# 0kam/alproj

Hardware: AMD Instinct MI355X
Metric: Gpoints/s projected (pinhole + Brown-Conrady, single pose) over the 100M-vertex DSM; CMA-ES iterations/s in `cma` (higher is better)
Workload: dtype f32

## Files before the change

### alproj_amd/csrc/alp_cma.hip

```cpp
#include "alp_points_internal.h"
#include "alp_sampler.h"

#include <cmath>

namespace {

using namespace alp;

constexpr int CMA_MAX_D = SAMPLER_MAX_D;
constexpr int CMA_MAX_P = 4096;
constexpr int CMA_MAX_STARTS = 1024;
constexpr int64_t CMA_MAX_TOTAL = 65536;
constexpr int TELL_THREADS = 256;
constexpr int JACOBI_MAX_SWEEPS = 40;
constexpr double CMA_EPS = 1e-8;
constexpr double CMA_SIGMA_MAX = 1e32;

struct CmaState {
    double mean[CMA_MAX_D], ps[CMA_MAX_D], pc[CMA_MAX_D], d[CMA_MAX_D];
    double C[CMA_MAX_D * CMA_MAX_D], B[CMA_MAX_D * CMA_MAX_D];
    double BD[CMA_MAX_D * CMA_MAX_D];
    double sigma;
    long long g;
    unsigned k0, k1;
};

struct CmaHyper {
    int D, P, mu, dmax, K;
    double mu_eff, c1, cmu, cc, c_sigma, d_sigma, chi_n, cm, sum_w;
};

struct ExpandArgs {
    double tmpl[ALP_NPARAM];
    double lo[CMA_MAX_D], hi[CMA_MAX_D];
    int idx[CMA_MAX_D];
    double origin[3];
};

template <typename T, int DMAX, bool LF>
__global__ __launch_bounds__(256) void cma_generation_kernel(SamplerArgs a0, ExpandArgs e, const CmaState *__restrict__ states, long long P,
                                                             long long total, double *__restrict__ x_out, double *__restrict__ cand_out,
                                                             PoseRec<T> *__restrict__ recs, long long lf_off) {
    const long long cand = ((long long)blockIdx.x * blockDim.x + threadIdx.x) >> 6;
    if (cand >= total) return;
    const long long start = cand / P, draw = cand - start * P;
    const CmaState *st = states + start;
    const int lane = (int)(threadIdx.x & 63);
    SamplerArgs a = a0;
#pragma unroll
    for (int i = 0; i < DMAX; ++i)
        if (i < a.D) a.mean[i] = st->mean[i];
    a.sigma = st->sigma;
    a.gen = (unsigned)st->g;
    a.k0 = st->k0;
    a.k1 = st->k1;
    const double *BD = st->BD;
    double z[DMAX], x[DMAX];
#pragma unroll
    for (int j = 0; j < DMAX; ++j) z[j] = 0.0;
    int accepted = -1;
    for (int base = 0; base < a.n_max && accepted < 0; base += 64) {
        const int t = base + lane;
        bool ok = false;
        if (t < a.n_max) {
            draw_normals<DMAX>(z, a.D, (unsigned)t, (unsigned)draw, a.gen, a.k0, a.k1);
            ok = make_x<DMAX, false>(a, BD, z, x);
        }
        const unsigned long long m = __ballot(ok);
        if (m) accepted = base + __ffsll((long long)m) - 1;
    }
    const int t_final = accepted >= 0 ? accepted : a.n_max;
    if (lane != (t_final & 63)) return;
    draw_normals<DMAX>(z, a.D, (unsigned)t_final, (unsigned)draw, a.gen, a.k0, a.k1);
    make_x<DMAX, true>(a, BD, z, x);
    double prm[ALP_NPARAM];
    for (int k = 0; k < ALP_NPARAM; ++k) prm[k] = e.tmpl[k];
#pragma unroll
    for (int i = 0; i < DMAX; ++i)
        if (i < a.D) {
            double xi = x[i];
            if (accepted < 0 && a.bounded) xi = fmin(fmax(xi, a.lower[i]), a.upper[i]);
            x_out[cand * a.D + i] = xi;
            prm[e.idx[i]] = xi * (e.hi[i] - e.lo[i]) + e.lo[i];
        }
    for (int k = 0; k < ALP_NPARAM; ++k) cand_out[cand * ALP_NPARAM + k] = prm[k];
    double g[POSE_WORDS];
    fold_pose_hd(prm, e.origin, g);
    for (int k = 0; k < POSE_WORDS; ++k) recs[cand].v[k] = (T)g[k];
    if (LF) {
        double lf[POSE_WORDS];
        lens_free_from_general_hd(g, lf);
        for (int k = 0; k < POSE_WORDS; ++k) recs[lf_off + cand].v[k] = (T)lf[k];
    }
}

__device__ __forceinline__ void circle_pair(int m, int r, int k, int *p, int *q) {
    const int a = k == 0 ? m - 1 : (r + k) % (m - 1);
    const int b = (r - k + (m - 1)) % (m - 1);
    *p = a < b ? a : b;
    *q = a < b ? b : a;
}

__device__ void jacobi_eigen(int D, double *C, double *B, double *d2, double *A, double *A2, double *V, double *V2, double *self_,
                             double *oth, double *dlt, int *partner, int *rotated, int *nrot) {
    const int tid = threadIdx.x;
    const int DD = D * D;
    for (int e = tid; e < DD; e += blockDim.x) {
        const int i = e / D, j = e % D;
        double s = 0;
        for (int k = 0; k < D; ++k) s += B[k * D + i] * B[k * D + j];
        A2[e] = s;
    }
    __syncthreads();
    for (int e = tid; e < DD; e += blockDim.x) {
        const int i = e / D, j = e % D;
        double s = 0;
        for (int k = 0; k < D; ++k) s += B[i * D + k] * ((k == j ? 1.5 : 0.0) - 0.5 * A2[k * D + j]);
        V2[e] = s;
    }
    __syncthreads();
    for (int e = tid; e < DD; e += blockDim.x) B[e] = V2[e];
    __syncthreads();
    for (int e = tid; e < DD; e += blockDim.x) {
        const int i = e / D, j = e % D;
        double s = 0;
        for (int k = 0; k < D; ++k) s += C[i * D + k] * B[k * D + j];
        A2[e] = s;
    }
    __syncthreads();
    for (int e = tid; e < DD; e += blockDim.x) {
        const int i = e / D, j = e % D;
        if (i <= j) {
            double s = 0;
            for (int k = 0; k < D; ++k) s += B[k * D + i] * A2[k * D + j];
            A[i * D + j] = s;
            A[j * D + i] = s;
        }
        V[e] = i == j ? 1.0 : 0.0;
    }
    __syncthreads();
    const int m = (D + 1) & ~1;
    for (int sweep = 0; sweep < JACOBI_MAX_SWEEPS && m >= 2; ++sweep) {
        if (tid == 0) *nrot = 0;
        __syncthreads();
        for (int r = 0; r < m - 1; ++r) {
            if (tid < m / 2) {
                int p, q;
                circle_pair(m, r, tid, &p, &q);
                if (q < D) {
                    const double app = A[p * D + p], aqq = A[q * D + q], apq = A[p * D + q];
                    const double g = 100.0 * fabs(apq);
                    double c = 1.0, s = 0.0, t = 0.0;
                    const bool rot = apq != 0.0 && !(fabs(app) + g == fabs(app) && fabs(aqq) + g == fabs(aqq));
                    if (rot) {
                        const double theta = (aqq - app) / (2.0 * apq);
                        if (fabs(theta) > 1e150) t = 0.5 / theta;
                        else {
                            t = 1.0 / (fabs(theta) + sqrt(theta * theta + 1.0));
                            if (theta < 0) t = -t;
                        }
                        c = 1.0 / sqrt(t * t + 1.0);
                        s = t * c;
                        *nrot = 1;
                    }
                    partner[p] = q; partner[q] = p;
                    self_[p] = c; self_[q] = c;
                    oth[p] = -s; oth[q] = s;
                    dlt[p] = -t * apq; dlt[q] = t * apq;
                    rotated[p] = rotated[q] = rot;
                } else if (p < D) {
                    partner[p] = p; self_[p] = 1.0; oth[p] = 0.0; dlt[p] = 0.0; rotated[p] = 0;
                }
            }
            __syncthreads();
            for (int e = tid; e < DD; e += blockDim.x) {
                const int i = e / D, j = e % D;
                double v;
                if (i == j) v = A[e] + dlt[i];
                else if (partner[i] == j && rotated[i]) v = 0.0;
                else {
                    const int lo = i < j ? i : j, hi = i < j ? j : i;
                    const int plo = partner[lo], phi = partner[hi];
                    v = self_[hi] * A[lo * D + hi];
                    if (oth[hi] != 0.0) v += oth[hi] * A[lo * D + phi];
                    v *= self_[lo];
                    if (oth[lo] != 0.0) {
                        double w = self_[hi] * A[plo * D + hi];
                        if (oth[hi] != 0.0) w += oth[hi] * A[plo * D + phi];
                        v += oth[lo] * w;
                    }
                }
                A2[e] = v;
                double u = V[i * D + j] * self_[j];
                if (oth[j] != 0.0) u += V[i * D + partner[j]] * oth[j];
                V2[e] = u;
            }
            __syncthreads();
            for (int e = tid; e < DD; e += blockDim.x) {
                A[e] = A2[e];
                V[e] = V2[e];
            }
            __syncthreads();
        }
        if (*nrot == 0) break;
        __syncthreads();
    }
    for (int e = tid; e < DD; e += blockDim.x) {
        const int i = e / D, j = e % D;
        double s = 0;
        for (int k = 0; k < D; ++k) s += B[i * D + k] * V[k * D + j];
        V2[e] = s;
    }
    for (int i = tid; i < D; i += blockDim.x) d2[i] = A[i * D + i];
    __syncthreads();
    for (int e = tid; e < DD; e += blockDim.x) B[e] = V2[e];
    __syncthreads();
}

template <bool TELL>
__global__ __launch_bounds__(TELL_THREADS) void cma_tell_kernel(CmaHyper h, CmaState *__restrict__ states, const double *__restrict__ weights,
                                                                const double *__restrict__ X_all, const double *__restrict__ sums_all,
                                                                const double *__restrict__ vals_all, double *__restrict__ loss_all,
                                                                int *__restrict__ order_all, double *__restrict__ ys_all,
                                                                double *__restrict__ wio_all) {
    const long long k = blockIdx.x, kP = k * h.P, kPD = kP * h.D;
    CmaState *__restrict__ st = states + k;
    const double *__restrict__ X = X_all + kPD;
    const double *__restrict__ sums = sums_all ? sums_all + kP : nullptr;
    const double n_total = sums_all ? sums_all[(long long)h.K * h.P] : 0.0;
    const double *__restrict__ vals = vals_all ? vals_all + kP : nullptr;
    double *__restrict__ loss_out = loss_all + kP;
    int *__restrict__ order_out = order_all + kP;
    double *__restrict__ ys = ys_all + kPD;
    double *__restrict__ wio = wio_all + kP;
    constexpr int M = CMA_MAX_D * CMA_MAX_D;
    __shared__ double C[M], B[M], A[M], A2[M], V[M], V2[M];
    __shared__ double mean[CMA_MAX_D], d[CMA_MAX_D], yw[CMA_MAX_D], ps[CMA_MAX_D], pc[CMA_MAX_D], d2[CMA_MAX_D];
    __shared__ double self_[CMA_MAX_D], oth[CMA_MAX_D], dlt[CMA_MAX_D];
    __shared__ int partner[CMA_MAX_D], rotated[CMA_MAX_D];
    __shared__ int nrot;
    __shared__ double sig, hsig;
    const int tid = threadIdx.x, D = h.D, P = h.P, DD = D * D;
    for (int e = tid; e < DD; e += blockDim.x) {
        C[e] = st->C[e];
        B[e] = st->B[e];
    }
    for (int i = tid; i < D; i += blockDim.x) {
        mean[i] = st->mean[i];
        d[i] = st->d[i];
        ps[i] = st->ps[i];
        pc[i] = st->pc[i];
    }
    if (tid == 0) sig = st->sigma;
    __syncthreads();
    if (TELL) {
        const long long g = st->g + 1;
        for (int i = tid; i < P; i += blockDim.x) loss_out[i] = vals ? vals[i] : sums[i] / n_total;
        __syncthreads();
        for (int i = tid; i < P; i += blockDim.x) {
            double ki = loss_out[i];
            if (ki != ki) ki = INFINITY;
            int r = 0;
            for (int j = 0; j < P; ++j) {
                double kj = loss_out[j];
                if (kj != kj) kj = INFINITY;
                r += (kj < ki) || (kj == ki && j < i);
            }
            order_out[r] = i;
        }
        __syncthreads();
        const double sigma = sig;
        for (int e = tid; e < P * D; e += blockDim.x) {
            const int r = e / D, j = e % D;
            ys[e] = (X[(long long)order_out[r] * D + j] - mean[j]) / sigma;
        }
        __syncthreads();
        for (int j = tid; j < D; j += blockDim.x) {
            double s = 0.0;
            for (int r = 0; r < h.mu; ++r) s = s + ys[(long long)r * D + j] * weights[r];
            yw[j] = s;
        }
        __syncthreads();
        const double cs = h.c_sigma, cmsig = h.cm * sigma;
        for (int e = tid; e < DD; e += blockDim.x) {
            const int i = e / D, j = e % D;
            double s = 0.0;
            for (int k = 0; k < D; ++k) s += (B[i * D + k] / d[k]) * B[j * D + k];
            A[e] = s;
        }
        for (int j = tid; j < D; j += blockDim.x) mean[j] = mean[j] + cmsig * yw[j];
        __syncthreads();
        const double sq_ps = sqrt(cs * (2.0 - cs) * h.mu_eff);
        for (int i = tid; i < D; i += blockDim.x) {
            double s = 0.0;
            for (int k = 0; k < D; ++k) s += A[i * D + k] * yw[k];
            ps[i] = (1.0 - cs) * ps[i] + sq_ps * s;
        }
        __syncthreads();
        if (tid == 0) {
            double nn = 0.0;
            for (int k = 0; k < D; ++k) nn += ps[k] * ps[k];
            const double norm_ps = sqrt(nn);
            double s2 = sig * exp((cs / h.d_sigma) * (norm_ps / h.chi_n - 1.0));
            sig = s2 < CMA_SIGMA_MAX ? s2 : CMA_SIGMA_MAX;
            const double h_left = norm_ps / sqrt(1.0 - pow(1.0 - cs, (double)(2 * (g + 1))));
            const double h_right = (1.4 + 2.0 / (double)(D + 1)) * h.chi_n;
            hsig = h_left < h_right ? 1.0 : 0.0;
        }
        __syncthreads();
        const double h_sigma = hsig, cc = h.cc;
        const double sq_pc = h_sigma * sqrt(cc * (2.0 - cc) * h.mu_eff);
        for (int i = tid; i < D; i += blockDim.x) pc[i] = (1.0 - cc) * pc[i] + sq_pc * yw[i];
        for (int r = tid; r < P; r += blockDim.x) {
            const double wr = weights[r];
            if (wr >= 0) {
                wio[r] = wr * 1.0;
            } else {
                double nn = 0.0;
                for (int i = 0; i < D; ++i) {
                    double s = 0.0;
                    for (int k = 0; k < D; ++k) s += ys[(long long)r * D + k] * A[i * D + k];
                    nn += s * s;
                }
                const double nrm = sqrt(nn);
                wio[r] = wr * ((double)D / (nrm * nrm + CMA_EPS));
            }
        }
        __syncthreads();
        const double delta_h = (1.0 - h_sigma) * cc * (2.0 - cc);
        const double c1 = h.c1, cmu = h.cmu;
        const double coef = 1.0 + c1 * delta_h - c1 - cmu * h.sum_w;
        for (int e = tid; e < DD; e += blockDim.x) {
            const int i = e / D, j = e % D;
            double rmu = 0.0;
            for (int r = 0; r < P; ++r) rmu += (ys[(long long)r * D + i] * wio[r]) * ys[(long long)r * D + j];
            A2[e] = coef * C[e] + c1 * (pc[i] * pc[j]) + cmu * rmu;
        }
        __syncthreads();
        for (int e = tid; e < DD; e += blockDim.x) C[e] = A2[e];
        if (tid == 0) st->g = g;
        __syncthreads();
    }
    for (int e = tid; e < DD; e += blockDim.x) {
        const int i = e / D, j = e % D;
        A2[e] = (C[i * D + j] + C[j * D + i]) / 2.0;
    }
    __syncthreads();
    for (int e = tid; e < DD; e += blockDim.x) C[e] = A2[e];
    __syncthreads();
    jacobi_eigen(D, C, B, d2, A, A2, V, V2, self_, oth, dlt, partner, rotated, &nrot);
    for (int i = tid; i < D; i += blockDim.x) d[i] = sqrt(d2[i] < 0 ? CMA_EPS : d2[i]);
    __syncthreads();
    for (int e = tid; e < DD; e += blockDim.x) {
        const int i = e / D, j = e % D;
        double s = 0.0;
        for (int k = 0; k < D; ++k) s += (B[i * D + k] * (d[k] * d[k])) * B[j * D + k];
        st->C[e] = s;
        st->B[e] = B[e];
    }
    for (int e = tid; e < h.dmax * h.dmax; e += blockDim.x) {
        const int i = e / h.dmax, j = e % h.dmax;
        st->BD[e] = (i < D && j < D) ? B[i * D + j] * d[j] : 0.0;
    }
    for (int i = tid; i < D; i += blockDim.x) {
        st->d[i] = d[i];
        if (TELL) {
            st->mean[i] = mean[i];
            st->ps[i] = ps[i];
            st->pc[i] = pc[i];
        }
    }
    if (TELL && tid == 0) st->sigma = sig;
}

}

struct alp_cma {
    alp_points *pts = nullptr;
    CmaHyper hy{};
    SamplerArgs sa{};
    ExpandArgs ex{};
    std::vector<uint64_t> seeds;
    bool lens_free = false, shared_pose = false;
    void *dev = nullptr;
    CmaState *st = nullptr;
    double *w = nullptr, *X = nullptr, *cand = nullptr, *loss = nullptr, *ys = nullptr, *wio = nullptr, *vals = nullptr;
    int *order = nullptr;
    bool pending = false;
    bool have_last = false;
    int64_t rows() const { return (int64_t)hy.K * hy.P; }
};

namespace alp {
void cma_points_gone(alp_cma_t *h) { h->pts = nullptr; }
}

namespace {

void fill_state(const alp_cma *h, int k, CmaState *s, const double *mean, double sigma, const double *C, const double *ps, const double *pc,
                int64_t g) {
    const int D = h->hy.D;
    memset(s, 0, sizeof(*s));
    for (int i = 0; i < D; ++i) {
        s->mean[i] = mean[i];
        s->ps[i] = ps[i];
        s->pc[i] = pc[i];
        s->d[i] = 1.0;
        s->B[i * D + i] = 1.0;
    }
    for (int e = 0; e < D * D; ++e) s->C[e] = C[e];
    s->sigma = sigma;
    s->g = g;
    s->k0 = (unsigned)h->seeds[(size_t)k];
    s->k1 = (unsigned)(h->seeds[(size_t)k] >> 32);
}

int upload_states(alp_cma *h, int k0, int n, const CmaState *s) {
    hipStream_t st = ctx().stream;
    ALP_HIP(hipMemcpyAsync(h->st + k0, s, (size_t)n * sizeof(CmaState), hipMemcpyHostToDevice, st));
    hipLaunchKernelGGL(cma_tell_kernel<false>, dim3(n), dim3(TELL_THREADS), 0, st, h->hy, h->st + k0, (const double *)h->w,
                       (const double *)h->X, (const double *)nullptr, (const double *)nullptr, h->loss, h->order, h->ys, h->wio);
    ALP_HIP(hipGetLastError());
    ALP_HIP(hipStreamSynchronize(st));
    return ALP_OK;
}

int usable(alp_cma *h, const char *what) {
    if (int rc = require_init()) return rc;
    if (!h) return fail(ALP_EINVAL, "%s: handle is NULL", what);
    if (h->pending) return fail(ALP_ESTATE, "%s: generations are enqueued; call alp_cma_wait first", what);
    return ALP_OK;
}

template <typename T, int DMAX>
void launch_generation(alp_cma *h, unsigned grid, hipStream_t st) {
    alp_points *p = h->pts;
    PoseRec<T> *recs = (PoseRec<T> *)p->cand_dev;
    if (h->lens_free)
        hipLaunchKernelGGL((cma_generation_kernel<T, DMAX, true>), dim3(grid), dim3(256), 0, st, h->sa, h->ex, (const CmaState *)h->st,
                           (long long)h->hy.P, (long long)h->rows(), h->X, h->cand, recs, (long long)p->cand_cap);
    else
        hipLaunchKernelGGL((cma_generation_kernel<T, DMAX, false>), dim3(grid), dim3(256), 0, st, h->sa, h->ex, (const CmaState *)h->st,
                           (long long)h->hy.P, (long long)h->rows(), h->X, h->cand, recs, (long long)p->cand_cap);
}

template <typename T>
void launch_generation_t(alp_cma *h, unsigned grid, hipStream_t st) {
    if (h->hy.dmax == 12) launch_generation<T, 12>(h, grid, st);
    else if (h->hy.dmax == 24) launch_generation<T, 24>(h, grid, st);
    else launch_generation<T, 32>(h, grid, st);
}

}

extern "C" {

int alp_cma_create_starts(alp_points_t *pts, const double tmpl[ALP_NPARAM], const int32_t *target_idx, int D, const double *lower,
                          const double *upper, int64_t P, int K, const double *weights, const double hyper[ALP_CMA_NHYPER],
                          int n_max_resampling, const uint64_t *seeds, alp_cma_t **out) {
    if (int rc = require_init()) return rc;
    ALP_REQUIRE(out, "out is NULL");
    *out = nullptr;
    ALP_REQUIRE(pts && tmpl && target_idx && lower && upper && weights && hyper && seeds, "NULL argument");
    ALP_REQUIRE(D >= 1 && D <= CMA_MAX_D, "D must be in [1, 32]");
    ALP_REQUIRE(P >= 1 && P <= CMA_MAX_P, "P must be in [1, 4096]");
    ALP_REQUIRE(K >= 1 && K <= CMA_MAX_STARTS, "K must be in [1, 1024]");
    ALP_REQUIRE((int64_t)K * P <= CMA_MAX_TOTAL, "K * P must be at most 65536");
    ALP_REQUIRE(n_max_resampling >= 0 && n_max_resampling <= (1 << 20), "n_max_resampling out of range");
    if (!pts->uo) return fail(ALP_ESTATE, "alp_cma_create: observed uv not set");
    for (int i = 0; i < D; ++i) {
        ALP_REQUIRE(target_idx[i] >= 0 && target_idx[i] < ALP_NPARAM, "target index out of range");
        ALP_REQUIRE(target_idx[i] != 21 && target_idx[i] != 22, "w and h cannot be targets (every candidate must share the image size)");
    }
    const int mu = (int)hyper[0];
    ALP_REQUIRE(mu >= 0 && mu <= P, "mu out of range");
    alp_cma *h = new alp_cma();
    h->pts = pts;
    const int dmax = D <= 12 ? 12 : (D <= 24 ? 24 : 32);
    h->hy = CmaHyper{D, (int)P, mu, dmax, K, hyper[1], hyper[2], hyper[3], hyper[4], hyper[5], hyper[6], hyper[7], hyper[8], hyper[9]};
    h->seeds.assign(seeds, seeds + K);
    memset(&h->sa, 0, sizeof(h->sa));
    for (int i = 0; i < D; ++i) {
        h->sa.lower[i] = 0.0;
        h->sa.upper[i] = 1.0;
    }
    h->sa.D = D;
    h->sa.n_max = n_max_resampling;
    h->sa.bounded = 1;
    memset(&h->ex, 0, sizeof(h->ex));
    for (int k = 0; k < ALP_NPARAM; ++k) h->ex.tmpl[k] = tmpl[k];
    for (int i = 0; i < D; ++i) {
        h->ex.idx[i] = target_idx[i];
        h->ex.lo[i] = lower[i];
        h->ex.hi[i] = upper[i];
    }
    memcpy(h->ex.origin, pts->origin, sizeof(h->ex.origin));
    bool lf = !getenv("ALP_POP_NO_LENS_FREE");
    for (int k = 9; k <= 20 && lf; ++k) lf = tmpl[k] == 0.0;
    for (int i = 0; i < D && lf; ++i) lf = !(target_idx[i] >= 9 && target_idx[i] <= 20);
    bool shared = P > 1 && !lf;
    for (int i = 0; i < D && shared; ++i) shared = target_idx[i] >= 7 && target_idx[i] <= 20;
    h->lens_free = lf;
    h->shared_pose = shared;
    const int64_t R = (int64_t)K * P;
    const size_t sz_state = round_up((int64_t)K * sizeof(CmaState), 256), sz_w = round_up(P * 8, 256), sz_p = round_up(R * 8, 256),
                 sz_pd = round_up(R * D * 8, 256), sz_cand = round_up(R * ALP_NPARAM * 8, 256), sz_ord = round_up(R * 4, 256);
    int rc = ALP_OK;
    if (hipMalloc(&h->dev, sz_state + sz_w + 3 * sz_p + 2 * sz_pd + sz_cand + sz_ord) != hipSuccess) rc = fail(ALP_EHIP, "alp_cma_create: hipMalloc failed");
    if (!rc) {
        char *q = (char *)h->dev;
        h->st = (CmaState *)q; q += sz_state;
        h->w = (double *)q; q += sz_w;
        h->loss = (double *)q; q += sz_p;
        h->wio = (double *)q; q += sz_p;
        h->vals = (double *)q; q += sz_p;
        h->X = (double *)q; q += sz_pd;
        h->ys = (double *)q; q += sz_pd;
        h->cand = (double *)q; q += sz_cand;
        h->order = (int *)q;
        if (hipMemcpy(h->w, weights, (size_t)P * 8, hipMemcpyHostToDevice) != hipSuccess) rc = fail(ALP_EHIP, "alp_cma_create: weights upload failed");
    }
    if (!rc) rc = points_pop_reserve(pts, R);
    if (!rc) {
        std::vector<double> mean(D, 0.5), C((size_t)D * D, 0.0), zero(D, 0.0);
        for (int i = 0; i < D; ++i) C[(size_t)i * D + i] = 1.0;
        std::vector<CmaState> s((size_t)K);
        for (int k = 0; k < K; ++k) fill_state(h, k, &s[(size_t)k], mean.data(), 1.0, C.data(), zero.data(), zero.data(), 0);
        rc = upload_states(h, 0, K, s.data());
    }
    if (rc) {
        if (h->dev) hipFree(h->dev);
        delete h;
        return rc;
    }
    pts->loops.push_back(h);
    *out = h;
    return ALP_OK;
}

int alp_cma_create(alp_points_t *pts, const double tmpl[ALP_NPARAM], const int32_t *target_idx, int D, const double *lower,
                   const double *upper, int64_t P, const double *weights, const double hyper[ALP_CMA_NHYPER], int n_max_resampling,
                   uint64_t seed, alp_cma_t **out) {
    return alp_cma_create_starts(pts, tmpl, target_idx, D, lower, upper, P, 1, weights, hyper, n_max_resampling, &seed, out);
}

int alp_cma_destroy(alp_cma_t *h) {
    if (!h) return ALP_OK;
    if (ctx().ready) hipStreamSynchronize(ctx().stream);
    if (h->pts) {
        h->pts->loop_pending = false;
        auto &v = h->pts->loops;
        for (size_t i = 0; i < v.size(); ++i)
            if (v[i] == h) {
                v.erase(v.begin() + (long)i);
                break;
            }
    }
    if (h->dev) hipFree(h->dev);
    delete h;
    return ALP_OK;
}

int alp_cma_set_state_at(alp_cma_t *h, int k, const double *mean, double sigma, const double *C, const double *p_sigma, const double *pc,
                         int64_t generation) {
    if (int rc = usable(h, "alp_cma_set_state")) return rc;
    ALP_REQUIRE(k >= 0 && k < h->hy.K, "start index out of range");
    ALP_REQUIRE(mean && C && p_sigma && pc, "NULL argument");
    ALP_REQUIRE(sigma > 0, "sigma must be positive");
    ALP_REQUIRE(generation >= 0, "generation is negative");
    CmaState s;
    fill_state(h, k, &s, mean, sigma, C, p_sigma, pc, generation);
    return upload_states(h, k, 1, &s);
}

int alp_cma_set_state(alp_cma_t *h, const double *mean, double sigma, const double *C, const double *p_sigma, const double *pc,
                      int64_t generation) {
    return alp_cma_set_state_at(h, 0, mean, sigma, C, p_sigma, pc, generation);
}

int alp_cma_get_state_at(alp_cma_t *h, int k, double *mean, double *sigma, double *C, double *p_sigma, double *pc, int64_t *generation,
                         double *B, double *Dvec) {
    if (int rc = usable(h, "alp_cma_get_state")) return rc;
    ALP_REQUIRE(k >= 0 && k < h->hy.K, "start index out of range");
    CmaState s;
    ALP_HIP(hipMemcpyAsync(&s, h->st + k, sizeof(s), hipMemcpyDeviceToHost, ctx().stream));
    ALP_HIP(hipStreamSynchronize(ctx().stream));
    const int D = h->hy.D;
    for (int i = 0; i < D; ++i) {
        if (mean) mean[i] = s.mean[i];
        if (p_sigma) p_sigma[i] = s.ps[i];
        if (pc) pc[i] = s.pc[i];
        if (Dvec) Dvec[i] = s.d[i];
    }
    for (int e = 0; e < D * D; ++e) {
        if (C) C[e] = s.C[e];
        if (B) B[e] = s.B[e];
    }
    if (sigma) *sigma = s.sigma;
    if (generation) *generation = s.g;
    return ALP_OK;
}

int alp_cma_get_state(alp_cma_t *h, double *mean, double *sigma, double *C, double *p_sigma, double *pc, int64_t *generation, double *B,
                      double *Dvec) {
    return alp_cma_get_state_at(h, 0, mean, sigma, C, p_sigma, pc, generation, B, Dvec);
}

int alp_cma_run(alp_cma_t *h, int64_t generations, int loss_kind, double f_scale) {
    if (int rc = usable(h, "alp_cma_run")) return rc;
    ALP_REQUIRE(generations >= 0, "generations is negative");
    ALP_REQUIRE(loss_kind == ALP_LOSS_MEAN_DIST || loss_kind == ALP_LOSS_HUBER, "unknown loss_kind");
    alp_points *p = h->pts;
    if (!p) return fail(ALP_ESTATE, "alp_cma_run: the point set of this device loop has been destroyed");
    if (p->pending_P > 0 || p->loop_pending)
        return fail(ALP_ESTATE, "alp_cma_run: the point set has an evaluation enqueued that has not been waited for");
    if (generations == 0) return ALP_OK;
    const int64_t R = h->rows();
    if (int rc = points_pop_reserve(p, R)) return rc;
    const unsigned grid = (unsigned)((R * 64 + 255) / 256);
    const bool batched = h->hy.K > 1;
    hipStream_t st = ctx().stream;
    h->pending = true;
    p->loop_pending = true;
    for (int64_t g = 0; g < generations; ++g) {
        if (p->precision == ALP_F64) launch_generation_t<double>(h, grid, st);
        else launch_generation_t<float>(h, grid, st);
        ALP_HIP(hipGetLastError());
        if (int rc = popeval_launch(p, R, loss_kind, f_scale, h->lens_free, h->shared_pose, batched, h->cand)) return rc;
        hipLaunchKernelGGL(cma_tell_kernel<true>, dim3(h->hy.K), dim3(TELL_THREADS), 0, st, h->hy, h->st, (const double *)h->w,
                           (const double *)h->X, (const double *)p->sums_dev, (const double *)nullptr, h->loss, h->order, h->ys, h->wio);
        ALP_HIP(hipGetLastError());
    }
    h->have_last = true;
    return ALP_OK;
}

int alp_cma_wait(alp_cma_t *h) {
    if (int rc = require_init()) return rc;
    ALP_REQUIRE(h, "handle is NULL");
    if (!h->pending) return fail(ALP_ESTATE, "alp_cma_wait: nothing enqueued");
    h->pending = false;
    if (h->pts) h->pts->loop_pending = false;
    ALP_HIP(hipStreamSynchronize(ctx().stream));
    return ALP_OK;
}

int alp_cma_tell_host(alp_cma_t *h, const double *X, const double *losses, int32_t *order_out) {
    if (int rc = usable(h, "alp_cma_tell_host")) return rc;
    ALP_REQUIRE(X && losses, "NULL argument");
    const int64_t R = h->rows(), D = h->hy.D;
    hipStream_t st = ctx().stream;
    ALP_HIP(hipMemcpyAsync(h->X, X, (size_t)(R * D) * 8, hipMemcpyHostToDevice, st));
    ALP_HIP(hipMemcpyAsync(h->vals, losses, (size_t)R * 8, hipMemcpyHostToDevice, st));
    hipLaunchKernelGGL(cma_tell_kernel<true>, dim3(h->hy.K), dim3(TELL_THREADS), 0, st, h->hy, h->st, (const double *)h->w,
                       (const double *)h->X, (const double *)nullptr, (const double *)h->vals, h->loss, h->order, h->ys, h->wio);
    ALP_HIP(hipGetLastError());
    if (order_out) ALP_HIP(hipMemcpyAsync(order_out, h->order, (size_t)R * 4, hipMemcpyDeviceToHost, st));
    ALP_HIP(hipStreamSynchronize(st));
    h->have_last = false;
    return ALP_OK;
}

int alp_cma_fetch_last(alp_cma_t *h, double *X, double *cand, double *losses) {
    if (int rc = usable(h, "alp_cma_fetch_last")) return rc;
    if (!h->have_last) return fail(ALP_ESTATE, "alp_cma_fetch_last: no device generation has run");
    const int64_t R = h->rows(), D = h->hy.D;
    hipStream_t st = ctx().stream;
    if (X) ALP_HIP(hipMemcpyAsync(X, h->X, (size_t)(R * D) * 8, hipMemcpyDeviceToHost, st));
    if (cand) ALP_HIP(hipMemcpyAsync(cand, h->cand, (size_t)R * ALP_NPARAM * 8, hipMemcpyDeviceToHost, st));
    if (losses) ALP_HIP(hipMemcpyAsync(losses, h->loss, (size_t)R * 8, hipMemcpyDeviceToHost, st));
    ALP_HIP(hipStreamSynchronize(st));
    return ALP_OK;
}

}
```

### alproj_amd/csrc/alp_sampler.h

```cpp
#pragma once

#include "alp_internal.h"

#include <cmath>

namespace alp {

constexpr int SAMPLER_MAX_D = 32;

__device__ __forceinline__ void philox4x32_10(unsigned c0, unsigned c1, unsigned c2, unsigned c3, unsigned k0, unsigned k1,
                                              unsigned out[4]) {
#pragma unroll
    for (int r = 0; r < 10; ++r) {
        const unsigned long long p0 = (unsigned long long)0xD2511F53u * c0, p1 = (unsigned long long)0xCD9E8D57u * c2;
        const unsigned n0 = (unsigned)(p1 >> 32) ^ c1 ^ k0, n1 = (unsigned)p1, n2 = (unsigned)(p0 >> 32) ^ c3 ^ k1, n3 = (unsigned)p0;
        c0 = n0; c1 = n1; c2 = n2; c3 = n3;
        k0 += 0x9E3779B9u;
        k1 += 0xBB67AE85u;
    }
    out[0] = c0; out[1] = c1; out[2] = c2; out[3] = c3;
}

template <int DMAX>
__device__ __forceinline__ void draw_normals(double (&z)[DMAX], int D, unsigned tr, unsigned cand, unsigned gen, unsigned k0, unsigned k1) {
#pragma unroll
    for (int j = 0; j < DMAX; j += 2) {
        if (j < D) {
            unsigned w[4];
            philox4x32_10((unsigned)(j >> 1), tr, cand, gen, k0, k1, w);
            const double u1 = ((double)(((unsigned long long)w[0] << 21) | (w[1] >> 11)) + 0.5) * (1.0 / 9007199254740992.0);
            const double u2 = ((double)(((unsigned long long)w[2] << 21) | (w[3] >> 11)) + 0.5) * (1.0 / 9007199254740992.0);
            const double rad = sqrt(-2.0 * log(u1)), ang = 6.283185307179586476925286766559 * u2;
            z[j] = rad * cos(ang);
            if (j + 1 < DMAX) z[j + 1] = (j + 1 < D) ? rad * sin(ang) : 0.0;
        }
    }
}

struct SamplerArgs {
    double mean[SAMPLER_MAX_D], lower[SAMPLER_MAX_D], upper[SAMPLER_MAX_D];
    double sigma;
    int D, n_max, bounded;
    unsigned k0, k1, gen;
};

template <int DMAX, bool KEEP>
__device__ __forceinline__ bool make_x(const SamplerArgs &a, const double *__restrict__ BD, const double (&z)[DMAX], double (&x)[DMAX]) {
    bool ok = true;
#pragma unroll
    for (int i = 0; i < DMAX; ++i) {
        if (i < a.D) {
            double y = 0.0;
#pragma unroll
            for (int j = 0; j < DMAX; ++j) y = fma(BD[i * DMAX + j], z[j], y);
            const double xi = fma(a.sigma, y, a.mean[i]);
            if (KEEP) x[i] = xi;
            if (a.bounded) ok = ok && xi >= a.lower[i] && xi <= a.upper[i];
        }
    }
    return ok;
}

}
```

### alproj_amd/csrc/alp_sampler.hip

```cpp
#include "alp_sampler.h"

namespace alp {

template <int DMAX>
__global__ __launch_bounds__(256) void cma_sample_kernel(SamplerArgs a, const double *__restrict__ BD, long long P,
                                                         double *__restrict__ x_out, int *__restrict__ tries_out) {
    const long long cand = ((long long)blockIdx.x * blockDim.x + threadIdx.x) >> 6;
    if (cand >= P) return;
    const int lane = (int)(threadIdx.x & 63);
    double z[DMAX], x[DMAX];
#pragma unroll
    for (int j = 0; j < DMAX; ++j) z[j] = 0.0;
    int accepted = -1;
    for (int base = 0; base < a.n_max && accepted < 0; base += 64) {
        const int t = base + lane;
        bool ok = false;
        if (t < a.n_max) {
            draw_normals<DMAX>(z, a.D, (unsigned)t, (unsigned)cand, a.gen, a.k0, a.k1);
            ok = make_x<DMAX, false>(a, BD, z, x);
        }
        const unsigned long long m = __ballot(ok);
        if (m) accepted = base + __ffsll((long long)m) - 1;
    }
    const int t_final = accepted >= 0 ? accepted : a.n_max;
    if (lane == (t_final & 63)) {
        draw_normals<DMAX>(z, a.D, (unsigned)t_final, (unsigned)cand, a.gen, a.k0, a.k1);
        make_x<DMAX, true>(a, BD, z, x);
#pragma unroll
        for (int i = 0; i < DMAX; ++i)
            if (i < a.D) {
                double xi = x[i];
                if (accepted < 0 && a.bounded) xi = fmin(fmax(xi, a.lower[i]), a.upper[i]);
                x_out[cand * a.D + i] = xi;
            }
        if (tries_out) tries_out[cand] = t_final;
    }
}

}

using namespace alp;

extern "C" int alp_cma_sample(const double *mean, double sigma, const double *BD, const double *lower, const double *upper,
                              int D, int64_t P, int n_max_resampling, uint64_t seed, uint64_t generation, double *x_out,
                              int32_t *tries_out) {
    if (int rc = require_init()) return rc;
    ALP_REQUIRE(mean && BD && x_out, "NULL argument");
    ALP_REQUIRE(D >= 1 && D <= SAMPLER_MAX_D, "D must be in [1, 32]");
    ALP_REQUIRE(P >= 1 && P <= (1 << 24), "P out of range");
    ALP_REQUIRE(n_max_resampling >= 0 && n_max_resampling <= (1 << 20), "n_max_resampling out of range");
    ALP_REQUIRE((lower == nullptr) == (upper == nullptr), "lower and upper must both be given or both be NULL");
    ALP_REQUIRE(sigma > 0, "sigma must be positive");
    SamplerArgs a;
    memset(&a, 0, sizeof(a));
    for (int i = 0; i < D; ++i) {
        a.mean[i] = mean[i];
        a.lower[i] = lower ? lower[i] : -INFINITY;
        a.upper[i] = upper ? upper[i] : INFINITY;
    }
    a.sigma = sigma;
    a.D = D;
    a.n_max = lower ? n_max_resampling : 1;
    if (a.n_max < 1) a.n_max = 0;
    a.bounded = lower != nullptr;
    a.k0 = (unsigned)seed;
    a.k1 = (unsigned)(seed >> 32);
    a.gen = (unsigned)generation;
    const int dmax = D <= 12 ? 12 : (D <= 24 ? 24 : 32);
    const size_t bd_bytes = (size_t)dmax * dmax * sizeof(double), x_bytes = (size_t)P * D * sizeof(double),
                 t_bytes = (size_t)P * sizeof(int);
    char *dev = nullptr;
    if (int rc = scratch_reserve(round_up((int64_t)bd_bytes, 256) + round_up((int64_t)x_bytes, 256) + t_bytes, (void **)&dev)) return rc;
    double *bd_dev = (double *)dev, *x_dev = (double *)(dev + round_up((int64_t)bd_bytes, 256));
    int *t_dev = (int *)((char *)x_dev + round_up((int64_t)x_bytes, 256));
    hipStream_t st = ctx().stream;
    double bd_pad[SAMPLER_MAX_D * SAMPLER_MAX_D];
    memset(bd_pad, 0, sizeof(bd_pad));
    for (int i = 0; i < D; ++i)
        for (int j = 0; j < D; ++j) bd_pad[i * dmax + j] = BD[i * D + j];
    ALP_HIP(hipMemcpyAsync(bd_dev, bd_pad, bd_bytes, hipMemcpyHostToDevice, st));
    const unsigned grid = (unsigned)((P * 64 + 255) / 256);
    int *tries_dev = tries_out ? t_dev : nullptr;
    if (dmax == 12) hipLaunchKernelGGL(cma_sample_kernel<12>, dim3(grid), dim3(256), 0, st, a, bd_dev, (long long)P, x_dev, tries_dev);
    else if (dmax == 24) hipLaunchKernelGGL(cma_sample_kernel<24>, dim3(grid), dim3(256), 0, st, a, bd_dev, (long long)P, x_dev, tries_dev);
    else hipLaunchKernelGGL(cma_sample_kernel<32>, dim3(grid), dim3(256), 0, st, a, bd_dev, (long long)P, x_dev, tries_dev);
    ALP_HIP(hipGetLastError());
    ALP_HIP(hipMemcpyAsync(x_out, x_dev, x_bytes, hipMemcpyDeviceToHost, st));
    if (tries_out) ALP_HIP(hipMemcpyAsync(tries_out, t_dev, t_bytes, hipMemcpyDeviceToHost, st));
    ALP_HIP(hipStreamSynchronize(st));
    return ALP_OK;
}
```

Measured before the change: 501.3.

## Parallelize CMA sampling per block and run eigen-solve on a single wave

Candidate sampling moves from one 64-lane wave per candidate to one block per candidate. The threads of that block generate Philox normal pairs for many resampling tries in parallel into shared memory, then one wave tests them for bounds acceptance and the accepting thread writes the result. The Jacobi eigendecomposition in the tell/update kernel now runs on a single wavefront, using wave barriers and ping-pong A/V buffers in place of block-wide syncs and copy-back passes. Part of the mean/ps/sigma update now runs on wave 0 while the other waves compute the negative-weight scaling. This is meant to cut serial RNG work and synchronisation cost, but it adds shared-memory traffic and larger blocks per candidate, and the eigen-solve now uses only 64 threads.

```diff
diff --git a/alproj_amd/csrc/alp_cma.hip b/alproj_amd/csrc/alp_cma.hip
--- a/alproj_amd/csrc/alp_cma.hip
+++ b/alproj_amd/csrc/alp_cma.hip
@@ -38,14 +38,16 @@
 };
 
 template <typename T, int DMAX, bool LF>
-__global__ __launch_bounds__(256) void cma_generation_kernel(SamplerArgs a0, ExpandArgs e, const CmaState *__restrict__ states, long long P,
-                                                             long long total, double *__restrict__ x_out, double *__restrict__ cand_out,
-                                                             PoseRec<T> *__restrict__ recs, long long lf_off) {
-    const long long cand = ((long long)blockIdx.x * blockDim.x + threadIdx.x) >> 6;
-    if (cand >= total) return;
+__global__ __launch_bounds__(DRAW_MAX_THREADS) void cma_generation_kernel(SamplerArgs a0, ExpandArgs e, const CmaState *__restrict__ states,
+                                                                          long long P, long long total, double *__restrict__ x_out,
+                                                                          double *__restrict__ cand_out, PoseRec<T> *__restrict__ recs,
+                                                                          long long lf_off) {
+    __shared__ double zs[DMAX * DRAW_TRIES];
+    __shared__ int acc;
+    __shared__ double prm[ALP_NPARAM];
+    const long long cand = blockIdx.x;
     const long long start = cand / P, draw = cand - start * P;
     const CmaState *st = states + start;
-    const int lane = (int)(threadIdx.x & 63);
     SamplerArgs a = a0;
 #pragma unroll
     for (int i = 0; i < DMAX; ++i)
@@ -54,32 +56,15 @@
     a.gen = (unsigned)st->g;
     a.k0 = st->k0;
     a.k1 = st->k1;
-    const double *BD = st->BD;
-    double z[DMAX], x[DMAX];
-#pragma unroll
-    for (int j = 0; j < DMAX; ++j) z[j] = 0.0;
-    int accepted = -1;
-    for (int base = 0; base < a.n_max && accepted < 0; base += 64) {
-        const int t = base + lane;
-        bool ok = false;
-        if (t < a.n_max) {
-            draw_normals<DMAX>(z, a.D, (unsigned)t, (unsigned)draw, a.gen, a.k0, a.k1);
-            ok = make_x<DMAX, false>(a, BD, z, x);
-        }
-        const unsigned long long m = __ballot(ok);
-        if (m) accepted = base + __ffsll((long long)m) - 1;
-    }
-    const int t_final = accepted >= 0 ? accepted : a.n_max;
-    if (lane != (t_final & 63)) return;
-    draw_normals<DMAX>(z, a.D, (unsigned)t_final, (unsigned)draw, a.gen, a.k0, a.k1);
-    make_x<DMAX, true>(a, BD, z, x);
-    double prm[ALP_NPARAM];
+    double x[DMAX];
+    int t_final;
+    if (!draw_candidate<DMAX>(a, st->BD, (unsigned)draw, zs, &acc, x, &t_final)) return;
     for (int k = 0; k < ALP_NPARAM; ++k) prm[k] = e.tmpl[k];
 #pragma unroll
     for (int i = 0; i < DMAX; ++i)
         if (i < a.D) {
             double xi = x[i];
-            if (accepted < 0 && a.bounded) xi = fmin(fmax(xi, a.lower[i]), a.upper[i]);
+            if (t_final == a.n_max && a.bounded) xi = fmin(fmax(xi, a.lower[i]), a.upper[i]);
             x_out[cand * a.D + i] = xi;
             prm[e.idx[i]] = xi * (e.hi[i] - e.lo[i]) + e.lo[i];
         }
@@ -101,57 +86,77 @@
     *q = a < b ? b : a;
 }
 
-__device__ void jacobi_eigen(int D, double *C, double *B, double *d2, double *A, double *A2, double *V, double *V2, double *self_,
-                             double *oth, double *dlt, int *partner, int *rotated, int *nrot) {
-    const int tid = threadIdx.x;
+__device__ __forceinline__ void wave_sync() {
+    __builtin_amdgcn_fence(__ATOMIC_RELEASE, "wavefront");
+    __builtin_amdgcn_wave_barrier();
+    __builtin_amdgcn_fence(__ATOMIC_ACQUIRE, "wavefront");
+}
+
+struct WaveElems {
+    int D, di, dj, i0, j0;
+    __device__ WaveElems(int D_, int lane) : D(D_), di(64 / D_), dj(64 % D_), i0(lane / D_), j0(lane % D_) {}
+    __device__ __forceinline__ void next(int *i, int *j) const {
+        *i += di;
+        *j += dj;
+        if (*j >= D) {
+            *j -= D;
+            *i += 1;
+        }
+    }
+};
+#define FOR_WAVE_ELEMS(w, lane, DD) for (int e = (lane), i = (w).i0, j = (w).j0; e < (DD); e += 64, (w).next(&i, &j))
+
+__device__ void jacobi_eigen_wave(int D, const double *C, double *B, double *d2, double *AA, double *VV, double *self_, double *oth,
+                                  double *dlt, int *partner, int *rotated) {
+    constexpr int M = CMA_MAX_D * CMA_MAX_D;
+    const int lane = threadIdx.x;
     const int DD = D * D;
-    for (int e = tid; e < DD; e += blockDim.x) {
-        const int i = e / D, j = e % D;
+    const WaveElems w(D, lane);
+    int ac = 0, an = M, vc = 0, vn = M;
+    FOR_WAVE_ELEMS(w, lane, DD) {
         double s = 0;
         for (int k = 0; k < D; ++k) s += B[k * D + i] * B[k * D + j];
-        A2[e] = s;
-    }
-    __syncthreads();
-    for (int e = tid; e < DD; e += blockDim.x) {
-        const int i = e / D, j = e % D;
+        AA[an + e] = s;
+    }
+    wave_sync();
+    FOR_WAVE_ELEMS(w, lane, DD) {
         double s = 0;
-        for (int k = 0; k < D; ++k) s += B[i * D + k] * ((k == j ? 1.5 : 0.0) - 0.5 * A2[k * D + j]);
-        V2[e] = s;
-    }
-    __syncthreads();
-    for (int e = tid; e < DD; e += blockDim.x) B[e] = V2[e];
-    __syncthreads();
-    for (int e = tid; e < DD; e += blockDim.x) {
-        const int i = e / D, j = e % D;
+        for (int k = 0; k < D; ++k) s += B[i * D + k] * ((k == j ? 1.5 : 0.0) - 0.5 * AA[an + k * D + j]);
+        VV[vn + e] = s;
+    }
+    wave_sync();
+    FOR_WAVE_ELEMS(w, lane, DD) B[e] = VV[vn + e];
+    wave_sync();
+    FOR_WAVE_ELEMS(w, lane, DD) {
         double s = 0;
         for (int k = 0; k < D; ++k) s += C[i * D + k] * B[k * D + j];
-        A2[e] = s;
-    }
-    __syncthreads();
-    for (int e = tid; e < DD; e += blockDim.x) {
-        const int i = e / D, j = e % D;
+        AA[an + e] = s;
+    }
+    wave_sync();
+    FOR_WAVE_ELEMS(w, lane, DD) {
         if (i <= j) {
             double s = 0;
-            for (int k = 0; k < D; ++k) s += B[k * D + i] * A2[k * D + j];
-            A[i * D + j] = s;
-            A[j * D + i] = s;
-        }
-        V[e] = i == j ? 1.0 : 0.0;
-    }
-    __syncthreads();
+            for (int k = 0; k < D; ++k) s += B[k * D + i] * AA[an + k * D + j];
+            AA[ac + i * D + j] = s;
+            AA[ac + j * D + i] = s;
+        }
+        VV[vc + e] = i == j ? 1.0 : 0.0;
+    }
+    wave_sync();
     const int m = (D + 1) & ~1;
     for (int sweep = 0; sweep < JACOBI_MAX_SWEEPS && m >= 2; ++sweep) {
-        if (tid == 0) *nrot = 0;
-        __syncthreads();
+        bool any = false;
         for (int r = 0; r < m - 1; ++r) {
-            if (tid < m / 2) {
+            const double *A = AA + ac;
+            bool rot = false;
+            if (lane < m / 2) {
                 int p, q;
-                circle_pair(m, r, tid, &p, &q);
+                circle_pair(m, r, lane, &p, &q);
                 if (q < D) {
                     const double app = A[p * D + p], aqq = A[q * D + q], apq = A[p * D + q];
                     const double g = 100.0 * fabs(apq);
                     double c = 1.0, s = 0.0, t = 0.0;
-                    const bool rot = apq != 0.0 && !(fabs(app) + g == fabs(app) && fabs(aqq) + g == fabs(aqq));
+                    rot = apq != 0.0 && !(fabs(app) + g == fabs(app) && fabs(aqq) + g == fabs(aqq));
                     if (rot) {
                         const double theta = (aqq - app) / (2.0 * apq);
                         if (fabs(theta) > 1e150) t = 0.5 / theta;
@@ -161,7 +166,6 @@
                         }
                         c = 1.0 / sqrt(t * t + 1.0);
                         s = t * c;
-                        *nrot = 1;
                     }
                     partner[p] = q; partner[q] = p;
                     self_[p] = c; self_[q] = c;
@@ -172,9 +176,10 @@
                     partner[p] = p; self_[p] = 1.0; oth[p] = 0.0; dlt[p] = 0.0; rotated[p] = 0;
                 }
             }
-            __syncthreads();
-            for (int e = tid; e < DD; e += blockDim.x) {
-                const int i = e / D, j = e % D;
+            any = any || __ballot(rot) != 0;
+            wave_sync();
+            const double *V = VV + vc;
+            FOR_WAVE_ELEMS(w, lane, DD) {
                 double v;
                 if (i == j) v = A[e] + dlt[i];
                 else if (partner[i] == j && rotated[i]) v = 0.0;
@@ -185,36 +190,31 @@
                     if (oth[hi] != 0.0) v += oth[hi] * A[lo * D + phi];
                     v *= self_[lo];
                     if (oth[lo] != 0.0) {
-                        double w = self_[hi] * A[plo * D + hi];
-                        if (oth[hi] != 0.0) w += oth[hi] * A[plo * D + phi];
-                        v += oth[lo] * w;
+                        double u = self_[hi] * A[plo * D + hi];
+                        if (oth[hi] != 0.0) u += oth[hi] * A[plo * D + phi];
+                        v += oth[lo] * u;
                     }
                 }
-                A2[e] = v;
+                AA[an + e] = v;
                 double u = V[i * D + j] * self_[j];
                 if (oth[j] != 0.0) u += V[i * D + partner[j]] * oth[j];
-                V2[e] = u;
-            }
-            __syncthreads();
-            for (int e = tid; e < DD; e += blockDim.x) {
-                A[e] = A2[e];
-                V[e] = V2[e];
-            }
-            __syncthreads();
-        }
-        if (*nrot == 0) break;
-        __syncthreads();
-    }
-    for (int e = tid; e < DD; e += blockDim.x) {
-        const int i = e / D, j = e % D;
+                VV[vn + e] = u;
+            }
+            wave_sync();
+            ac ^= an; an ^= ac; ac ^= an;
+            vc ^= vn; vn ^= vc; vc ^= vn;
+        }
+        if (!any) break;
+    }
+    FOR_WAVE_ELEMS(w, lane, DD) {
         double s = 0;
-        for (int k = 0; k < D; ++k) s += B[i * D + k] * V[k * D + j];
-        V2[e] = s;
-    }
-    for (int i = tid; i < D; i += blockDim.x) d2[i] = A[i * D + i];
-    __syncthreads();
-    for (int e = tid; e < DD; e += blockDim.x) B[e] = V2[e];
-    __syncthreads();
+        for (int k = 0; k < D; ++k) s += B[i * D + k] * VV[vc + k * D + j];
+        VV[vn + e] = s;
+    }
+    for (int i = lane; i < D; i += 64) d2[i] = AA[ac + i * D + i];
+    wave_sync();
+    FOR_WAVE_ELEMS(w, lane, DD) B[e] = VV[vn + e];
+    wave_sync();
 }
 
 template <bool TELL>
@@ -234,15 +234,15 @@
     double *__restrict__ ys = ys_all + kPD;
     double *__restrict__ wio = wio_all + kP;
     constexpr int M = CMA_MAX_D * CMA_MAX_D;
-    __shared__ double C[M], B[M], A[M], A2[M], V[M], V2[M];
+    __shared__ double C[M], B[M], AA[2 * M], VV[2 * M];
     __shared__ double mean[CMA_MAX_D], d[CMA_MAX_D], yw[CMA_MAX_D], ps[CMA_MAX_D], pc[CMA_MAX_D], d2[CMA_MAX_D];
     __shared__ double self_[CMA_MAX_D], oth[CMA_MAX_D], dlt[CMA_MAX_D];
     __shared__ int partner[CMA_MAX_D], rotated[CMA_MAX_D];
-    __shared__ int nrot;
     __shared__ double sig, hsig;
+    double *A = AA, *A2 = AA + M;
     const int tid = threadIdx.x, D = h.D, P = h.P, DD = D * D;
     for (int e = tid; e < DD; e += blockDim.x) {
-        C[e] = st->C[e];
+        (TELL ? C : A2)[e] = st->C[e];
         B[e] = st->B[e];
     }
     for (int i = tid; i < D; i += blockDim.x) {
@@ -252,7 +252,6 @@
         pc[i] = st->pc[i];
     }
     if (tid == 0) sig = st->sigma;
-    __syncthreads();
     if (TELL) {
         const long long g = st->g + 1;
         for (int i = tid; i < P; i += blockDim.x) loss_out[i] = vals ? vals[i] : sums[i] / n_total;
@@ -274,59 +273,62 @@
             const int r = e / D, j = e % D;
             ys[e] = (X[(long long)order_out[r] * D + j] - mean[j]) / sigma;
         }
-        __syncthreads();
-        for (int j = tid; j < D; j += blockDim.x) {
-            double s = 0.0;
-            for (int r = 0; r < h.mu; ++r) s = s + ys[(long long)r * D + j] * weights[r];
-            yw[j] = s;
-        }
-        __syncthreads();
-        const double cs = h.c_sigma, cmsig = h.cm * sigma;
         for (int e = tid; e < DD; e += blockDim.x) {
             const int i = e / D, j = e % D;
             double s = 0.0;
             for (int k = 0; k < D; ++k) s += (B[i * D + k] / d[k]) * B[j * D + k];
             A[e] = s;
         }
-        for (int j = tid; j < D; j += blockDim.x) mean[j] = mean[j] + cmsig * yw[j];
         __syncthreads();
-        const double sq_ps = sqrt(cs * (2.0 - cs) * h.mu_eff);
-        for (int i = tid; i < D; i += blockDim.x) {
-            double s = 0.0;
-            for (int k = 0; k < D; ++k) s += A[i * D + k] * yw[k];
-            ps[i] = (1.0 - cs) * ps[i] + sq_ps * s;
+        const double cs = h.c_sigma, cc = h.cc;
+        if (tid < 64) {
+            const double cmsig = h.cm * sigma;
+            for (int j = tid; j < D; j += 64) {
+                double s = 0.0;
+                for (int r = 0; r < h.mu; ++r) s = s + ys[(long long)r * D + j] * weights[r];
+                yw[j] = s;
+            }
+            wave_sync();
+            const double sq_ps = sqrt(cs * (2.0 - cs) * h.mu_eff);
+            for (int i = tid; i < D; i += 64) {
+                mean[i] = mean[i] + cmsig * yw[i];
+                double s = 0.0;
+                for (int k = 0; k < D; ++k) s += A[i * D + k] * yw[k];
+                ps[i] = (1.0 - cs) * ps[i] + sq_ps * s;
+            }
+            wave_sync();
+            if (tid == 0) {
+                double nn = 0.0;
+                for (int k = 0; k < D; ++k) nn += ps[k] * ps[k];
+                const double norm_ps = sqrt(nn);
+                double s2 = sig * exp((cs / h.d_sigma) * (norm_ps / h.chi_n - 1.0));
+                sig = s2 < CMA_SIGMA_MAX ? s2 : CMA_SIGMA_MAX;
+                const double h_left = norm_ps / sqrt(1.0 - pow(1.0 - cs, (double)(2 * (g + 1))));
+                const double h_right = (1.4 + 2.0 / (double)(D + 1)) * h.chi_n;
+                hsig = h_left < h_right ? 1.0 : 0.0;
+            }
+            wave_sync();
+            const double sq_pc = hsig * sqrt(cc * (2.0 - cc) * h.mu_eff);
+            for (int i = tid; i < D; i += 64) pc[i] = (1.0 - cc) * pc[i] + sq_pc * yw[i];
+        } else {
+            for (int r = tid - 64; r < P; r += blockDim.x - 64) {
+                const double wr = weights[r];
+                if (wr >= 0) {
+                    wio[r] = wr * 1.0;
+                } else {
+                    double nn = 0.0;
+                    for (int i = 0; i < D; ++i) {
+                        double s = 0.0;
+                        for (int k = 0; k < D; ++k) s += ys[(long long)r * D + k] * A[i * D + k];
+                        nn += s * s;
+                    }
+                    const double nrm = sqrt(nn);
+                    wio[r] = wr * ((double)D / (nrm * nrm + CMA_EPS));
+                }
+            }
         }
         __syncthreads();
-        if (tid == 0) {
-            double nn = 0.0;
-            for (int k = 0; k < D; ++k) nn += ps[k] * ps[k];
-            const double norm_ps = sqrt(nn);
-            double s2 = sig * exp((cs / h.d_sigma) * (norm_ps / h.chi_n - 1.0));
-            sig = s2 < CMA_SIGMA_MAX ? s2 : CMA_SIGMA_MAX;
-            const double h_left = norm_ps / sqrt(1.0 - pow(1.0 - cs, (double)(2 * (g + 1))));
-            const double h_right = (1.4 + 2.0 / (double)(D + 1)) * h.chi_n;
-            hsig = h_left < h_right ? 1.0 : 0.0;
-        }
-        __syncthreads();
-        const double h_sigma = hsig, cc = h.cc;
-        const double sq_pc = h_sigma * sqrt(cc * (2.0 - cc) * h.mu_eff);
-        for (int i = tid; i < D; i += blockDim.x) pc[i] = (1.0 - cc) * pc[i] + sq_pc * yw[i];
-        for (int r = tid; r < P; r += blockDim.x) {
-            const double wr = weights[r];
-            if (wr >= 0) {
-                wio[r] = wr * 1.0;
-            } else {
-                double nn = 0.0;
-                for (int i = 0; i < D; ++i) {
-                    double s = 0.0;
-                    for (int k = 0; k < D; ++k) s += ys[(long long)r * D + k] * A[i * D + k];
-                    nn += s * s;
-                }
-                const double nrm = sqrt(nn);
-                wio[r] = wr * ((double)D / (nrm * nrm + CMA_EPS));
-            }
-        }
-        __syncthreads();
+        const double h_sigma = hsig;
         const double delta_h = (1.0 - h_sigma) * cc * (2.0 - cc);
         const double c1 = h.c1, cmu = h.cmu;
         const double coef = 1.0 + c1 * delta_h - c1 - cmu * h.sum_w;
@@ -336,20 +338,16 @@
             for (int r = 0; r < P; ++r) rmu += (ys[(long long)r * D + i] * wio[r]) * ys[(long long)r * D + j];
             A2[e] = coef * C[e] + c1 * (pc[i] * pc[j]) + cmu * rmu;
         }
-        __syncthreads();
-        for (int e = tid; e < DD; e += blockDim.x) C[e] = A2[e];
         if (tid == 0) st->g = g;
-        __syncthreads();
-    }
-    for (int e = tid; e < DD; e += blockDim.x) {
-        const int i = e / D, j = e % D;
-        A2[e] = (C[i * D + j] + C[j * D + i]) / 2.0;
     }
     __syncthreads();
-    for (int e = tid; e < DD; e += blockDim.x) C[e] = A2[e];
-    __syncthreads();
-    jacobi_eigen(D, C, B, d2, A, A2, V, V2, self_, oth, dlt, partner, rotated, &nrot);
-    for (int i = tid; i < D; i += blockDim.x) d[i] = sqrt(d2[i] < 0 ? CMA_EPS : d2[i]);
+    if (tid < 64) {
+        const WaveElems w(D, tid);
+        FOR_WAVE_ELEMS(w, tid, DD) C[e] = (A2[i * D + j] + A2[j * D + i]) / 2.0;
+        wave_sync();
+        jacobi_eigen_wave(D, C, B, d2, AA, VV, self_, oth, dlt, partner, rotated);
+        for (int i = tid; i < D; i += 64) d[i] = sqrt(d2[i] < 0 ? CMA_EPS : d2[i]);
+    }
     __syncthreads();
     for (int e = tid; e < DD; e += blockDim.x) {
         const int i = e / D, j = e % D;
@@ -437,10 +435,10 @@
     alp_points *p = h->pts;
     PoseRec<T> *recs = (PoseRec<T> *)p->cand_dev;
     if (h->lens_free)
-        hipLaunchKernelGGL((cma_generation_kernel<T, DMAX, true>), dim3(grid), dim3(256), 0, st, h->sa, h->ex, (const CmaState *)h->st,
+        hipLaunchKernelGGL((cma_generation_kernel<T, DMAX, true>), dim3(grid), dim3((unsigned)draw_block_threads(h->hy.D)), 0, st, h->sa, h->ex, (const CmaState *)h->st,
                            (long long)h->hy.P, (long long)h->rows(), h->X, h->cand, recs, (long long)p->cand_cap);
     else
-        hipLaunchKernelGGL((cma_generation_kernel<T, DMAX, false>), dim3(grid), dim3(256), 0, st, h->sa, h->ex, (const CmaState *)h->st,
+        hipLaunchKernelGGL((cma_generation_kernel<T, DMAX, false>), dim3(grid), dim3((unsigned)draw_block_threads(h->hy.D)), 0, st, h->sa, h->ex, (const CmaState *)h->st,
                            (long long)h->hy.P, (long long)h->rows(), h->X, h->cand, recs, (long long)p->cand_cap);
 }
 
@@ -617,7 +615,7 @@
     if (generations == 0) return ALP_OK;
     const int64_t R = h->rows();
     if (int rc = points_pop_reserve(p, R)) return rc;
-    const unsigned grid = (unsigned)((R * 64 + 255) / 256);
+    const unsigned grid = (unsigned)R;
     const bool batched = h->hy.K > 1;
     hipStream_t st = ctx().stream;
     h->pending = true;
diff --git a/alproj_amd/csrc/alp_sampler.h b/alproj_amd/csrc/alp_sampler.h
--- a/alproj_amd/csrc/alp_sampler.h
+++ b/alproj_amd/csrc/alp_sampler.h
@@ -21,20 +21,15 @@
     out[0] = c0; out[1] = c1; out[2] = c2; out[3] = c3;
 }
 
-template <int DMAX>
-__device__ __forceinline__ void draw_normals(double (&z)[DMAX], int D, unsigned tr, unsigned cand, unsigned gen, unsigned k0, unsigned k1) {
-#pragma unroll
-    for (int j = 0; j < DMAX; j += 2) {
-        if (j < D) {
-            unsigned w[4];
-            philox4x32_10((unsigned)(j >> 1), tr, cand, gen, k0, k1, w);
-            const double u1 = ((double)(((unsigned long long)w[0] << 21) | (w[1] >> 11)) + 0.5) * (1.0 / 9007199254740992.0);
-            const double u2 = ((double)(((unsigned long long)w[2] << 21) | (w[3] >> 11)) + 0.5) * (1.0 / 9007199254740992.0);
-            const double rad = sqrt(-2.0 * log(u1)), ang = 6.283185307179586476925286766559 * u2;
-            z[j] = rad * cos(ang);
-            if (j + 1 < DMAX) z[j + 1] = (j + 1 < D) ? rad * sin(ang) : 0.0;
-        }
-    }
+__device__ __forceinline__ void draw_pair(unsigned pair, unsigned tr, unsigned cand, unsigned gen, unsigned k0, unsigned k1, double *z0,
+                                          double *z1) {
+    unsigned w[4];
+    philox4x32_10(pair, tr, cand, gen, k0, k1, w);
+    const double u1 = ((double)(((unsigned long long)w[0] << 21) | (w[1] >> 11)) + 0.5) * (1.0 / 9007199254740992.0);
+    const double u2 = ((double)(((unsigned long long)w[2] << 21) | (w[3] >> 11)) + 0.5) * (1.0 / 9007199254740992.0);
+    const double rad = sqrt(-2.0 * log(u1)), ang = 6.283185307179586476925286766559 * u2;
+    *z0 = rad * cos(ang);
+    *z1 = rad * sin(ang);
 }
 
 struct SamplerArgs {
@@ -61,4 +56,48 @@
     return ok;
 }
 
+constexpr int DRAW_TRIES = 64;
+constexpr int DRAW_MAX_THREADS = 512;
+
+__host__ __device__ inline int draw_tries_per_pass(int D) {
+    const int np = (D + 1) / 2, tp = DRAW_MAX_THREADS / np;
+    return tp < DRAW_TRIES ? tp : DRAW_TRIES;
 }
+inline int draw_block_threads(int D) { return (draw_tries_per_pass(D) * ((D + 1) / 2) + 63) & ~63; }
+
+template <int DMAX>
+__device__ __forceinline__ bool draw_candidate(const SamplerArgs &a, const double *__restrict__ BD, unsigned cand, double *zs, int *acc,
+                                               double (&x)[DMAX], int *t_final) {
+    const int th = (int)threadIdx.x, np = (a.D + 1) >> 1, tp = draw_tries_per_pass(a.D);
+    const int pair = th / tp, tl = th - pair * tp;
+    int accepted = -1, base = 0;
+    for (;;) {
+        const int t = base + tl;
+        if (pair < np && t <= a.n_max) {
+            double z0, z1;
+            draw_pair((unsigned)pair, (unsigned)t, cand, a.gen, a.k0, a.k1, &z0, &z1);
+            zs[(2 * pair) * DRAW_TRIES + tl] = z0;
+            if (2 * pair + 1 < DMAX) zs[(2 * pair + 1) * DRAW_TRIES + tl] = z1;
+        }
+        __syncthreads();
+        if (th < 64) {
+            bool ok = false;
+            if (th < tp && base + th <= a.n_max) {
+                double z[DMAX];
+#pragma unroll
+                for (int j = 0; j < DMAX; ++j) z[j] = j < a.D ? zs[j * DRAW_TRIES + th] : 0.0;
+                ok = make_x<DMAX, true>(a, BD, z, x) && base + th < a.n_max;
+            }
+            const unsigned long long m = __ballot(ok);
+            if (th == 0) *acc = m ? base + __ffsll((long long)m) - 1 : -1;
+        }
+        __syncthreads();
+        accepted = *acc;
+        if (accepted >= 0 || base + tp > a.n_max) break;
+        base += tp;
+    }
+    *t_final = accepted >= 0 ? accepted : a.n_max;
+    return th == *t_final - base;
+}
+
+}
diff --git a/alproj_amd/csrc/alp_sampler.hip b/alproj_amd/csrc/alp_sampler.hip
--- a/alproj_amd/csrc/alp_sampler.hip
+++ b/alproj_amd/csrc/alp_sampler.hip
@@ -3,38 +3,22 @@
 namespace alp {
 
 template <int DMAX>
-__global__ __launch_bounds__(256) void cma_sample_kernel(SamplerArgs a, const double *__restrict__ BD, long long P,
-                                                         double *__restrict__ x_out, int *__restrict__ tries_out) {
-    const long long cand = ((long long)blockIdx.x * blockDim.x + threadIdx.x) >> 6;
-    if (cand >= P) return;
-    const int lane = (int)(threadIdx.x & 63);
-    double z[DMAX], x[DMAX];
+__global__ __launch_bounds__(DRAW_MAX_THREADS) void cma_sample_kernel(SamplerArgs a, const double *__restrict__ BD, long long P,
+                                                                      double *__restrict__ x_out, int *__restrict__ tries_out) {
+    __shared__ double zs[DMAX * DRAW_TRIES];
+    __shared__ int acc;
+    const long long cand = blockIdx.x;
+    double x[DMAX];
+    int t_final;
+    if (!draw_candidate<DMAX>(a, BD, (unsigned)cand, zs, &acc, x, &t_final)) return;
 #pragma unroll
-    for (int j = 0; j < DMAX; ++j) z[j] = 0.0;
-    int accepted = -1;
-    for (int base = 0; base < a.n_max && accepted < 0; base += 64) {
-        const int t = base + lane;
-        bool ok = false;
-        if (t < a.n_max) {
-            draw_normals<DMAX>(z, a.D, (unsigned)t, (unsigned)cand, a.gen, a.k0, a.k1);
-            ok = make_x<DMAX, false>(a, BD, z, x);
+    for (int i = 0; i < DMAX; ++i)
+        if (i < a.D) {
+            double xi = x[i];
+            if (t_final == a.n_max && a.bounded) xi = fmin(fmax(xi, a.lower[i]), a.upper[i]);
+            x_out[cand * a.D + i] = xi;
         }
-        const unsigned long long m = __ballot(ok);
-        if (m) accepted = base + __ffsll((long long)m) - 1;
-    }
-    const int t_final = accepted >= 0 ? accepted : a.n_max;
-    if (lane == (t_final & 63)) {
-        draw_normals<DMAX>(z, a.D, (unsigned)t_final, (unsigned)cand, a.gen, a.k0, a.k1);
-        make_x<DMAX, true>(a, BD, z, x);
-#pragma unroll
-        for (int i = 0; i < DMAX; ++i)
-            if (i < a.D) {
-                double xi = x[i];
-                if (accepted < 0 && a.bounded) xi = fmin(fmax(xi, a.lower[i]), a.upper[i]);
-                x_out[cand * a.D + i] = xi;
-            }
-        if (tries_out) tries_out[cand] = t_final;
-    }
+    if (tries_out) tries_out[cand] = t_final;
 }
 
 }
@@ -79,11 +63,11 @@
     for (int i = 0; i < D; ++i)
         for (int j = 0; j < D; ++j) bd_pad[i * dmax + j] = BD[i * D + j];
     ALP_HIP(hipMemcpyAsync(bd_dev, bd_pad, bd_bytes, hipMemcpyHostToDevice, st));
-    const unsigned grid = (unsigned)((P * 64 + 255) / 256);
+    const unsigned grid = (unsigned)P, block = (unsigned)draw_block_threads(D);
     int *tries_dev = tries_out ? t_dev : nullptr;
-    if (dmax == 12) hipLaunchKernelGGL(cma_sample_kernel<12>, dim3(grid), dim3(256), 0, st, a, bd_dev, (long long)P, x_dev, tries_dev);
-    else if (dmax == 24) hipLaunchKernelGGL(cma_sample_kernel<24>, dim3(grid), dim3(256), 0, st, a, bd_dev, (long long)P, x_dev, tries_dev);
-    else hipLaunchKernelGGL(cma_sample_kernel<32>, dim3(grid), dim3(256), 0, st, a, bd_dev, (long long)P, x_dev, tries_dev);
+    if (dmax == 12) hipLaunchKernelGGL(cma_sample_kernel<12>, dim3(grid), dim3(block), 0, st, a, bd_dev, (long long)P, x_dev, tries_dev);
+    else if (dmax == 24) hipLaunchKernelGGL(cma_sample_kernel<24>, dim3(grid), dim3(block), 0, st, a, bd_dev, (long long)P, x_dev, tries_dev);
+    else hipLaunchKernelGGL(cma_sample_kernel<32>, dim3(grid), dim3(block), 0, st, a, bd_dev, (long long)P, x_dev, tries_dev);
     ALP_HIP(hipGetLastError());
     ALP_HIP(hipMemcpyAsync(x_out, x_dev, x_bytes, hipMemcpyDeviceToHost, st));
     if (tries_out) ALP_HIP(hipMemcpyAsync(tries_out, t_dev, t_bytes, hipMemcpyDeviceToHost, st));
```

Result: no change. 501.6 (median of 2 runs) (+0.1%).
